# beautifulNow1992/bolt

Hardware: AMD Instinct MI355X
Metric: swap/transpose GB/s + stat-reduce GB/s, % of HBM/xGMI roofline, 1-8 GPUs (higher is better)
Workload: dtype f32; 1 GPU; C2 f32 (2000,512,512)/GPU key=time: swap((0,),(0,1)) + mean/std(axis=2); split=1, parallelism=dp1, collectives=none

## Files before the change

bolt_amd/csrc/bm_copy.hip:

```cpp
#include "bm_common.h"
#include "bm_wave.h"
#include "../../include/bolt_mi355x.h"

#include <algorithm>
#include <cstdlib>
#include <type_traits>
#include <vector>

namespace {

constexpr int kThreads = 256;
constexpr int kRcThreads = 256;
constexpr int kUnroll = 1;
constexpr uint64_t kRcGridCap = 16777208;
constexpr int64_t kDiagMinStep = 65536;
constexpr int64_t kDiagMaxRow = 4096;
constexpr int kPkTA = 128, kPkTB = 512, kPkThreads = 1024;
constexpr int kGenGridCap = 4096;
constexpr int kASpread = 32;
constexpr int64_t kRunsMaxBytes = 64;
constexpr uint64_t kMaxGrid = 0xffffffffull / 1024;

struct Diag16 {
  int on;
// ... 36 lines not shown
        const uint64_t v = g - row * vpr.d;
        int64_t so, dof;
        decomp_n<ND>(dg.on ? diag16_row(row, dg) : row, d, so, dof);
        reg[u] = __builtin_nontemporal_load(reinterpret_cast<const V *>(src + so + (int64_t)v * VB));
        doff[u] = dof + (int64_t)v * VB;
      }
    }
#pragma unroll
    for (int u = 0; u < kUnroll; ++u) {
      if (doff[u] >= 0) __builtin_nontemporal_store(reg[u], reinterpret_cast<V *>(dst + doff[u]));
    }
  }
}

struct TransDesc {
  int64_t La;
  int64_t Lb;
  int64_t sb;
  int64_t da;
  FastDiv ntB;
  FastDiv ntAB;
  uint64_t ntiles;
  Decomp batch;
  FastDiv Lb1, La1;
  int64_t sb2, da2;
  FastDiv asp;
  uint64_t aspq;
};

template <bool FUSED>
__device__ __forceinline__ int64_t brow(const TransDesc &d, int64_t b) {
  if (!FUSED) return b * d.sb;
  const int64_t hi = (int64_t)fd_div((uint64_t)b, d.Lb1);
  return (b - hi * (int64_t)d.Lb1.d) * d.sb + hi * d.sb2;
}

template <bool FUSED>
__device__ __forceinline__ int64_t arow(const TransDesc &d, int64_t a) {
  if (!FUSED) return a * d.da;
  const int64_t hi = (int64_t)fd_div((uint64_t)a, d.La1);
  return (a - hi * (int64_t)d.La1.d) * d.da + hi * d.da2;
}


struct MomOut {
  double *parts;
  int64_t nrows;
  int64_t pitch;
};
struct NoMom {};

__device__ __forceinline__ double pair_fold16(double a, double b, int lane) {
  const bool hi = lane & 8;
  double v = (hi ? b : a) + dpp_mov<0x140>(hi ? a : b);
  v += dpp_mov<0x141>(v);
  v += dpp_mov<0x4E>(v);
  v += dpp_mov<0xB1>(v);
  return v;
}

template <typename T, int TA, int TB, int VA, int VB, bool FUSED = false, typename F = void>
__global__ void __launch_bounds__(kThreads)
    k_transpose(const T *__restrict__ src, T *__restrict__ dst, TransDesc d,
                typename std::conditional<std::is_void<F>::value, NoMom, MomOut>::type mo) {
  __shared__ T tile[TB][TA + 1];
  constexpr int NVA = TA / VA;
  constexpr int RPA = kThreads / NVA;
  constexpr int NVB = TB / VB;
  constexpr int RPB = kThreads / NVB;
  static_assert(NVA <= kThreads && NVB <= kThreads, "tile row wider than the block");
  static_assert(RPA <= TB && RPB <= TA && TB % RPA == 0 && TA % RPB == 0, "tile too small for the thread layout");
  constexpr int NL = TB / RPA;
  constexpr int NS = TA / RPB;
  constexpr int RPL = (VA * (int)sizeof(T) + 3) / 4;
  constexpr int NLB = (NL * RPL <= 64) ? NL : (16 / RPL > 0 ? 16 / RPL : 1);
  static_assert(NL % NLB == 0, "load batch must divide the loads");
  const int tx = threadIdx.x % NVA, ty = threadIdx.x / NVA;
  const int ux = threadIdx.x % NVB, uy = threadIdx.x / NVB;
  const int ia = tx * VA;
  const int ib = ux * VB;
  constexpr bool MOM = !std::is_void<F>::value;
  constexpr int NSEG = NVB / 16;
  static_assert(!MOM || (!FUSED && sizeof(typename std::conditional<MOM, F, T>::type) == sizeof(T) &&
                         VA * sizeof(T) == 16 && VB * sizeof(T) == 16 && NVB % 16 == 0 && NS % 2 == 0 &&
                         3 * TA <= kThreads),
                "moments: vectorised unfused tiles of float / double only");
  __shared__ double mst[MOM ? (2 * NSEG + 1) * TA : 1];
  double p1 = 0.0, p2 = 0.0, pK = 0.0;

  for (uint64_t t = blockIdx.x; t < d.ntiles; t += gridDim.x) {
    const uint64_t bt = fd_div(t, d.ntAB);
    const uint64_t rem = t - bt * d.ntAB.d;
    uint64_t ta = fd_div(rem, d.ntB);
    uint64_t tb = rem - ta * d.ntB.d;
    if (d.asp.d > 1) {
      const uint64_t hi = fd_div(ta, d.asp);
      ta = (ta - hi * d.asp.d) * d.aspq + hi;
    }
    int64_t so, dof;
    decomp_le4(bt, d.batch, so, dof);
    const int64_t a0 = (int64_t)ta * TA, b0 = (int64_t)tb * TB;

    const T *s = src + so + a0;
    const bool fullA = (a0 + ia + VA <= d.La);
#pragma unroll
    for (int i0 = 0; i0 < NL; i0 += NLB) {
      T v[NLB][VA];
#pragma unroll
      for (int j = 0; j < NLB; ++j) {
        const int rb = ty + (i0 + j) * RPA;
        if (b0 + rb < d.Lb) {
          const T *p = s + ia + brow<FUSED>(d, b0 + rb);
          if (fullA) {
            vload_nt<T, VA>(p, v[j]);
          } else {
#pragma unroll
            for (int k = 0; k < VA; ++k) v[j][k] = (a0 + ia + k < d.La) ? p[k] : T(0);
          }
        }
      }
#pragma unroll
      for (int j = 0; j < NLB; ++j) {
        const int rb = ty + (i0 + j) * RPA;
#pragma unroll
        for (int k = 0; k < VA; ++k) tile[rb][ia + k] = v[j][k];
      }
    }
    __syncthreads();

    T *q = dst + b0;
    if constexpr (!MOM) q += dof;
    const bool fullB = (b0 + ib + VB <= d.Lb);
#pragma unroll
    for (int it = 0; it < NS; ++it) {
      const int ra = uy + it * RPB;
      if (MOM || a0 + ra < d.La) {
        T w[VB];
#pragma unroll
        for (int k = 0; k < VB; ++k) w[k] = tile[ib + k][ra];
        if (!MOM || a0 + ra < d.La) {
          T *p = q + ib;
          if constexpr (MOM) p += (dof + (a0 + ra) * d.da) * mo.pitch;
          else p += arow<FUSED>(d, a0 + ra);
          if (fullB) {
            vstore_nt<T, VB>(p, w);
          } else {
#pragma unroll
            for (int k = 0; k < VB; ++k)
              if (b0 + ib + k < d.Lb) p[k] = w[k];
          }
        }
        if constexpr (MOM) {
          const double K0 = (double)__builtin_bit_cast(F, tile[0][ra]);
          const double K = K0 - K0 == 0.0 ? K0 : 0.0;
          double s1 = 0.0, s2 = 0.0;
#pragma unroll
          for (int k = 0; k < VB; ++k) {
            const double y = b0 + ib + k < d.Lb ? (double)__builtin_bit_cast(F, w[k]) - K : 0.0;
            s1 += y;
            s2 = fma(y, y, s2);
          }
          if ((it & 1) == 0) {
            p1 = s1;
            p2 = s2;
            pK = K;
          } else {
            const int lane = threadIdx.x & 63;
            s1 = pair_fold16(p1, s1, lane);
            s2 = pair_fold16(p2, s2, lane);
            if ((lane & 7) == 0) {
              const int rr = (lane & 8) ? ra : ra - RPB, seg = ux / 16;
              mst[rr * NSEG + seg] = s1;
              mst[(TA + rr) * NSEG + seg] = s2;
              if (seg == 0) mst[2 * TA * NSEG + rr] = (lane & 8) ? K : pK;
            }
          }
        }
      }
    }
    __syncthreads();
    if constexpr (MOM) {
      const int r = threadIdx.x % TA, plane = threadIdx.x / TA;
      if (plane < 3 && a0 + r < d.La) {
        double S1 = 0.0, S2 = 0.0;
#pragma unroll
        for (int g = 0; g < NSEG; ++g) {
          S1 += mst[r * NSEG + g];
          S2 += mst[(TA + r) * NSEG + g];
        }
        const double n = (double)min((int64_t)TB, d.Lb - b0);
        const double m1 = S1 / n;
        const double m2 = fma(-S1, m1, S2);
        const int64_t row = dof + (a0 + r) * d.da;
        mo.parts[((int64_t)tb * 3 + plane) * mo.nrows + row] =
            plane == 0 ? mst[2 * TA * NSEG + r] : plane == 1 ? m1 : (m2 > 0.0 ? m2 : 0.0);
      }
    }
  }
}


template <typename T, int TA, int TB, int NT = kThreads>
__global__ void __launch_bounds__(NT)
    k_transpose_pk(const T *__restrict__ src, T *__restrict__ dst, TransDesc d) {
  constexpr int P = 4 / (int)sizeof(T);
  constexpr int VA = 16 / (int)sizeof(T);
  constexpr int TBW = TB / P;
  constexpr int NVA = TA / VA;
  constexpr int RGA = NT / NVA;
  constexpr int NL = TBW / RGA;
  constexpr int NVB = TBW / 4;
  constexpr int RPB = NT / NVB;
  constexpr int NS = TA / RPB;
  constexpr int BITS = 8 * (int)sizeof(T);
  static_assert(NL >= 1 && TBW % RGA == 0 && NS >= 1 && TA % RPB == 0, "tile too small for the thread layout");
  static_assert(NL * P * 4 <= 64, "loads in flight exceed the register budget");
  __shared__ uint32_t tile[TBW][TA + 1];
  const int tx = threadIdx.x % NVA, ty = threadIdx.x / NVA;
  const int ux = threadIdx.x % NVB, uy = threadIdx.x / NVB;
  const int ia = tx * VA;

  for (uint64_t t = blockIdx.x; t < d.ntiles; t += gridDim.x) {
    const uint64_t bt = fd_div(t, d.ntAB);
    const uint64_t rem = t - bt * d.ntAB.d;
    const uint64_t ta = fd_div(rem, d.ntB);
    uint64_t tb = rem - ta * d.ntB.d;
    int64_t so, dof;
    decomp_le4(bt, d.batch, so, dof);
    const int64_t a0 = (int64_t)ta * TA, b0 = (int64_t)tb * TB;

    const T *s = src + so + a0 + b0 * d.sb;
// ... 858 lines not shown
```

bolt_amd/csrc/bm_reduce.hip:

```cpp
#include "bm_common.h"
#include "bm_wave.h"
#include "../../include/bolt_mi355x.h"

#include <cmath>

namespace {

constexpr int kThreads = 256;
constexpr int64_t kMaxBlocks = 0xffffffffLL / kThreads;
constexpr int kColsUnroll = 8;
constexpr int64_t kColsBlocks = 2048;
constexpr int64_t kColsTcv = 64;
constexpr int64_t kColsTcvMin = 64;
constexpr int kRowsUnroll = 2;
constexpr int kIntUnroll = 8;

enum Mode {
  M_MEAN = 0, M_MOM = 1, M_FSUM = 2, M_ISUM = 3, M_OR = 4, M_MAX = 5, M_MIN = 6,
  M_FPROD = 7, M_IPROD = 8, M_LAND = 9, M_BAND = 10, M_BOR = 11, M_BXOR = 12, M_FMAX = 13, M_FMIN = 14,
  M_MEANMOM = 15
};
template <int MODE> constexpr bool mean_part() { return MODE == M_MEAN || MODE == M_MEANMOM; }
template <int MODE> constexpr bool mom_part() { return MODE == M_MOM || MODE == M_MEANMOM; }

// ... 193 lines not shown
  if (na == nb) {
    f = 0.5;
  } else {
    f = nb / n;
  }
  ma = fma(delta, f, ma);
  if (need_m2) qa = qa + qb + delta * delta * (na * f);
  na = n;
}

__device__ __forceinline__ void store_out(void *out, int64_t idx, double v, int dt) {
  switch (dt) {
    case BM_F16: ((_Float16 *)out)[idx] = (_Float16)v; break;
    case BM_F32: ((float *)out)[idx] = (float)v; break;
    default: ((double *)out)[idx] = v; break;
  }
}

__device__ __forceinline__ void store_int(void *out, int64_t idx, uint64_t v, int dt) {
  switch (dt) {
    case BM_BOOL:
    case BM_U8:
    case BM_I8: ((uint8_t *)out)[idx] = (uint8_t)v; break;
    case BM_U16:
    case BM_I16:
    case BM_F16: ((uint16_t *)out)[idx] = (uint16_t)v; break;
    case BM_U32:
    case BM_I32:
    case BM_F32: ((uint32_t *)out)[idx] = (uint32_t)v; break;
    default: ((uint64_t *)out)[idx] = v; break;
  }
}

__device__ __forceinline__ double finish(int stat, double mean, double m2, double n) {
  if (stat == BM_STAT_MEAN) return mean;
  const double var = n > 0.0 ? m2 / n : __builtin_nan("");
  return stat == BM_STAT_VAR ? var : sqrt(var);
}

constexpr int kFinalMoments = 2;
struct Sink {
  void *out;
  int out_dtype;
  int stat;
  int final_out;
  double *p0;
  double *p1;
  double *p2;
  int shifted;
  void *om, *ov, *os;
  double *k0, *k1;
};

__device__ __forceinline__ void emit_kept(const Sink &sk, int64_t idx, double mean_y, double m2, double P) {
  sk.k0[idx] = P + mean_y;
  sk.k1[idx] = m2 > 0.0 ? m2 : 0.0;
}

__device__ __forceinline__ void emit_mom(const Sink &sk, int64_t idx, int64_t e, int64_t c, double n,
                                         double mean_y, double m2, double P) {
  m2 = m2 > 0.0 ? m2 : 0.0;
  if (sk.k0) emit_kept(sk, idx, mean_y, m2, P);
  if (sk.final_out == kFinalMoments) {
    if (sk.om) store_out(sk.om, idx, n > 0.0 ? P + mean_y : 0.0, sk.out_dtype);
    if (sk.ov) store_out(sk.ov, idx, finish(BM_STAT_VAR, 0.0, m2, n), sk.out_dtype);
    if (sk.os) store_out(sk.os, idx, finish(BM_STAT_STD, 0.0, m2, n), sk.out_dtype);
    return;
  }
  if (sk.final_out) {
    store_out(sk.out, idx, finish(sk.stat, 0.0, m2, n), sk.out_dtype);
    return;
  }
  sk.p0[idx] = sk.shifted ? mean_y : P + mean_y;
  sk.p1[idx] = m2;
  if (sk.shifted && c == 0) sk.p2[e] = P;
}

template <int MODE>
__device__ __forceinline__ void emit(const Sink &sk, int64_t e, double n, double mean, double m2,
                                     uint64_t u) {
  if (bit_mode<MODE>()) {
    if (sk.final_out) store_int(sk.out, e, u, sk.out_dtype);
    else ((uint64_t *)sk.p0)[e] = u;
  } else if (facc_mode<MODE>()) {
    if (sk.final_out) store_out(sk.out, e, mean, sk.out_dtype);
    else sk.p0[e] = mean;
  } else {
    if (sk.final_out) store_out(sk.out, e, finish(sk.stat, mean, m2, n), sk.out_dtype);
    else {
      sk.p0[e] = mean;
      if (MODE == M_MOM) sk.p1[e] = m2;
    }
  }
}

__device__ __forceinline__ uint64_t xcd_block() {
  uint64_t bid = blockIdx.x;
  const uint64_t g8 = gridDim.x / 8 * 8;
  if (bid < g8) bid = (bid % 8) * (g8 / 8) + bid / 8;
  return bid;
}

struct ColsDesc {
  int64_t O, R, I;
  int64_t rchunk;
  int64_t nchunks;
  int32_t tcv;
  int32_t nph;
  FastDiv ntc;
  int64_t tile0;
};

template <typename T, int VEC, int MODE>
__global__ void __launch_bounds__(kThreads)
// ... 1005 lines not shown
  if (p.nchunks <= 1) {
    int rc = launch_main(mode, dt, p, src, O, R, P, I, sk, st);
    if (rc) return rc;
    return check_launch(who);
  }
  const size_t need = ws_bytes_for(mode, p, nout);
  if (!ws || ws_bytes < need) {
    bm_set_error("%s: workspace too small (%zu < %zu)", who, ws_bytes, need);
    return BM_E_WS;
  }
  double *w0 = (double *)ws;
  double *w1 = w0 + (size_t)p.nchunks * nout;
  Sink part = sk;
  part.final_out = 0;
  part.p0 = w0;
  part.p1 = w1;
  part.p2 = w1 + (size_t)p.nchunks * nout;
  part.shifted = mode == M_MOM;
  int rc = launch_main(mode, dt, p, src, O, R, P, I, part, st);
  if (rc) return rc;
  CombDesc cd{};
  cd.nout = nout;
  cd.nparts = p.nchunks;
  cd.part_stride = nout;
  cd.R = R;
  cd.rchunk = p.rchunk;
  cd.explicit_counts = 0;
  cd.int_sums = mode == M_MOM && !is_float(dt) && dtype_size(dt) <= 2;
  cd.pivots = mode == M_MOM && !cd.int_sums;
  rc = launch_combine(mode, dt, w0, w1, cd, sk, st);
  if (rc) return rc;
  return check_launch(who);
}

__global__ void __launch_bounds__(kThreads)
    k_red_merge_tiles(const double *__restrict__ parts, int64_t nparts, int64_t tb, int64_t R, int64_t nrows,
                      double *__restrict__ state) {
  const int64_t step = (int64_t)gridDim.x * kThreads;
  for (int64_t e = (int64_t)blockIdx.x * kThreads + threadIdx.x; e < nrows; e += step) {
    const double K0 = parts[e];
    double n = 0.0, m = 0.0, q = 0.0;
    for (int64_t p = 0; p < nparts; ++p) {
      const double nb = (double)(min(R, (p + 1) * tb) - p * tb);
      const double *pp = parts + 3 * p * nrows + e;
      chan(n, m, q, nb, (pp[0] - K0) + pp[nrows], pp[2 * nrows], true);
    }
    m += K0;
    if (m != m) {
      double s = 0.0;
      for (int64_t p = 0; p < nparts; ++p) s += parts[3 * p * nrows + e] + parts[(3 * p + 1) * nrows + e];
      m = s;
    }
    state[e] = m;
    state[nrows + e] = q > 0.0 ? q : 0.0;
  }
}

}

int bm_merge_tile_moments(const double *parts, int64_t nparts, int64_t tb, int64_t R, int64_t nrows,
                          double *state, hipStream_t stream) {
  int64_t g = cdiv(nrows, kThreads);
  if (g > 4096) g = 4096;
  k_red_merge_tiles<<<(int)g, kThreads, 0, stream>>>(parts, nparts, tb, R, nrows, state);
  return check_launch("bm_copy_strided_moments");
}

extern "C" int bm_reduce_workspace_bytes(int stat, int in_dtype, int64_t O, int64_t R, int64_t I,
                                         size_t *bytes) {
  if (!bytes) { bm_set_error("bm_reduce_workspace_bytes: null out"); return BM_E_ARG; }
  int rc = check_args(stat, in_dtype, O, R, I, "bm_reduce_workspace_bytes");
  if (rc) return rc;
  const int mode = mode_of(stat, in_dtype);
  const size_t a = ws_bytes_for(mode, plan_reduce(in_dtype, O, R, I, nullptr, R), O * I);
  const size_t b = ws_bytes_for(mode, plan_reduce(in_dtype, O, R, I, (const void *)1, R), O * I);
  *bytes = a > b ? a : b;
  return BM_OK;
}

namespace {
int reduce_to_out(int stat, const void *src, int in_dtype, int64_t O, int64_t R, int64_t I, int64_t P,
                  void *out, int out_dtype, void *workspace, size_t workspace_bytes, void *stream,
                  const char *who) {
  int rc = check_args(stat, in_dtype, O, R, I, who);
  if (rc) return rc;
  if (!src || !out) { bm_set_error("%s: null pointer", who); return BM_E_ARG; }
  const int mode = mode_of(stat, in_dtype);
  if (!out_dtype_ok(stat, mode, in_dtype, out_dtype)) {
    bm_set_error("%s: out_dtype %d does not fit stat %d on dtype %d (float for statistics and "
                 "float sums / products, bool for logical and / or, else the input dtype)",
                 who, out_dtype, stat, in_dtype);
    return BM_E_ARG;
  }
  if (is_float(in_dtype) && (mode == M_BAND || mode == M_BOR || mode == M_BXOR)) {
    bm_set_error("%s: bitwise reductions need an integer or bool dtype", who);
    return BM_E_ARG;
  }
  Sink sk{};
  sk.out = out;
  sk.out_dtype = out_dtype;
  sk.stat = stat;
  sk.final_out = 1;
  return run_reduce(stat, src, in_dtype, O, R, I, sk, workspace, workspace_bytes,
                    (hipStream_t)stream, who, P);
}
}

// ... 185 lines not shown
```

bolt_amd/csrc/bm_wave.h:

```cpp
#pragma once

#include "bm_common.h"

template <typename T> __device__ __forceinline__ double to_f64(T x) { return (double)x; }
template <> __device__ __forceinline__ double to_f64<_Float16>(_Float16 x) { return (double)(float)x; }

template <int CTRL, typename V> __device__ __forceinline__ V dpp_mov(V v) {
  static_assert(sizeof(V) == 8, "64-bit lane values");
  const uint64_t u = __builtin_bit_cast(uint64_t, v);
  const uint32_t lo = (uint32_t)__builtin_amdgcn_update_dpp(0, (int)(uint32_t)u, CTRL, 0xf, 0xf, false);
  const uint32_t hi = (uint32_t)__builtin_amdgcn_update_dpp(0, (int)(uint32_t)(u >> 32), CTRL, 0xf, 0xf, false);
  return __builtin_bit_cast(V, ((uint64_t)hi << 32) | lo);
}
template <typename V, typename F> __device__ __forceinline__ V wave_fold(V v, int lane, F op) {
  V p = dpp_mov<0xB1>(v);
  v = (lane & 1) ? op(p, v) : op(v, p);
  p = dpp_mov<0x4E>(v);
  v = (lane & 2) ? op(p, v) : op(v, p);
  p = dpp_mov<0x141>(v);
  v = (lane & 4) ? op(p, v) : op(v, p);
  p = dpp_mov<0x140>(v);
  v = (lane & 8) ? op(p, v) : op(v, p);
  p = dpp_mov<0x142>(v);
  if (lane & 16) v = op(p, v);
  p = dpp_mov<0x143>(v);
  if (lane & 32) v = op(p, v);
  return v;
}
constexpr int kFoldLane = 63;
template <int L> __device__ __forceinline__ double lane_of(double v) {
  const uint64_t u = __builtin_bit_cast(uint64_t, v);
  const uint32_t lo = (uint32_t)__builtin_amdgcn_readlane((int)(uint32_t)u, L);
  const uint32_t hi = (uint32_t)__builtin_amdgcn_readlane((int)(uint32_t)(u >> 32), L);
  return __builtin_bit_cast(double, ((uint64_t)hi << 32) | lo);
}
__device__ __forceinline__ double lane0_of(double v) { return lane_of<0>(v); }

constexpr uint64_t kRedXcdSkew = 37;
__device__ __forceinline__ uint64_t rows_block() {
  uint64_t bid = blockIdx.x;
  const uint64_t g8 = gridDim.x / 8 * 8;
  if (bid < g8) {
    const uint64_t E = g8 / 8;
    bid = (bid % 8) * E + (bid / 8 + (bid % 8) * kRedXcdSkew) % E;
  }
  return bid;
}
```

bolt_amd/mi355x/array.py:

```python
import collections
import functools
import os

import numpy as np

from bolt_amd.mi355x import _lib, reduction
from bolt_amd.mi355x._ops import backend_for, dtype_code
from bolt_amd.base import BoltArray
from bolt_amd.mi355x.context import local_shape
from bolt_amd.mi355x.dist import all_gather_bytes, concat_rows_sharded, gather_to_host, permute_sharded, redistribute_rows, select_sharded, _empty
from bolt_amd.mi355x.transfer import to_device, to_host
from bolt_amd.local import BoltArrayLocal
from bolt_amd.mi355x.plan import getplan, check_plan, padded_strides, swap_perm, swap_shape, reduce_layout
from bolt_amd.utils import tupleize, argpack, inshape, istransposeable, isreshapeable

_STAT_CODES = {'mean': _lib.STAT_MEAN, 'variance': _lib.STAT_VAR, 'stdev': _lib.STAT_STD}


def _ufunc_stats():
    import operator
    return {operator.add: _lib.STAT_SUM, np.add: _lib.STAT_SUM,
            np.maximum: _lib.STAT_MAX, np.minimum: _lib.STAT_MIN,
            operator.mul: _lib.STAT_PROD, np.multiply: _lib.STAT_PROD,
            np.logical_and: _lib.STAT_LAND, np.logical_or: _lib.STAT_LOR,
# ... 86 lines not shown
    if rows < 2:
        return None
    sstr = [1] * len(shape)
    for k in range(len(shape) - 2, -1, -1):
        sstr[k] = sstr[k + 1] * shape[k + 1]
    return P, rows, list(new_shape), [sstr[p] for p in perm], _padded_strides(new_shape, P)


_DEVICE_BYTES = {}


def _pitch_fits(pp, es, device):
    if device.type != "cuda":
        return True
    import torch
    P, rows, oshape = pp[0], pp[1], pp[2]
    need = rows * (P + oshape[-1]) * es
    idx = device.index if device.index is not None else torch.cuda.current_device()
    total = _DEVICE_BYTES.get(idx)
    if total is None:
        total = _DEVICE_BYTES[idx] = torch.cuda.get_device_properties(idx).total_memory
    if need * 8 <= total:
        return True
    free = torch.cuda.mem_get_info(idx)[0] + torch.cuda.memory_reserved(idx) - torch.cuda.memory_allocated(idx)
    return need <= free


_padded_strides = padded_strides


@functools.lru_cache(maxsize=1024)
def _aligned_vshape_of(shape, split, axis):
    tokeys = [a - split for a in axis if a >= split]
    tovalues = [a for a in range(split) if a not in axis]
    if not (tokeys or tovalues):
        return None
    ref = swap_shape(shape, split, tovalues, tokeys)
    if ref is None:
        return None
    vs = ref[0][ref[1]:]
    kept = tuple(d for i, d in enumerate(shape) if i not in set(axis))
    return None if vs == kept else vs


KEEP_MOMENTS = os.environ.get("BOLT_AMD_KEEP_MOMENTS", "1") != "0"
_KEEP_MIN_BYTES = 256 << 20
_KEEP_STATE_DIV = 64
_KEEP_COLS = False

FUSE_SWAP_MOMENTS = os.environ.get("BOLT_AMD_FUSE_SWAP_MOMENTS", "1") != "0"
_FUSE_SWAP_MIN_BYTES = 256 << 20
_FUSE_SWAP_STATE_DIV = 64

Kept = collections.namedtuple('Kept', ('state', 'count', 'nlaunch', 'drop', 'serves_mean'))

Stats = collections.namedtuple('Stats', ('count', 'mean', 'var', 'std'))
_STATS_FIELDS = reduction.STATS_FIELDS
_STATS_NAMES = {'mean': 'mean', 'var': 'var', 'variance': 'var', 'std': 'std', 'stdev': 'std'}
_STAT_AXES = {}


class BoltArrayMI355X(BoltArray):

    _metadata = {
        '_shape': None,
        '_split': None,
        '_dtype': None,
        '_ordered': True,
    }

    def __init__(self, data, shape=None, split=None, dtype=None, ordered=True, context=None,
                 npartitions=None):
        self._data = data
        self._shape = tuple(int(s) for s in shape)
        self._split = int(split)
        self._dtype = np.dtype(dtype)
        self._mode = 'mi355x'
        self._ordered = ordered
        self._ctx = context
        self._npartitions = npartitions

    @property
    def _constructor(self):
        return BoltArrayMI355X

    @classmethod
    def _ingest(cls, arry, permutation, shape, split, dtype, ctx, npartitions):
        import torch
        dev = ctx.device
        es = dtype.itemsize
        arry = np.ascontiguousarray(arry)
        identity = list(permutation) == list(range(len(shape)))
        lo, hi = ctx.local_bounds(shape[0])
        rowbytes = int(np.prod(shape[1:], dtype=np.int64)) * es
        if identity:
            data = to_device(arry[lo:hi].reshape(-1).view(np.uint8), dev)
        elif ctx.world_size == 1:
            full = to_device(arry.reshape(-1).view(np.uint8), dev)
            data = _empty(full.numel(), dev)
            if full.numel():
                backend_for(dev).permute(full, arry.shape, permutation, es, data)
        else:
            pshape = tuple(arry.shape[i] for i in permutation)
            inner0 = int(np.prod(pshape[1:], dtype=np.int64))
            s0, e0 = lo * (rowbytes // es), hi * (rowbytes // es)
            if e0 == s0 or inner0 == 0:
                data = _empty(0, dev)
# ... 159 lines not shown
                sstr = [pstr[p] for p in perm]
            else:
                src, sstr = self._data, None
            be = backend_for(src.device)
            R = new_shape[-1]
            if pp is not None:
                P, rows, oshape, psstr, dstr = pp
            else:
                P, oshape, dstr = R, list(new_shape), _padded_strides(new_shape, R)
                if sstr is None:
                    cstr = _padded_strides(self._shape, self._shape[-1])
                    psstr = [cstr[p] for p in perm]
            csstr = psstr if sstr is None else sstr
            st = self._swap_state(be, src.device, new_shape, es, oshape, csstr, dstr, P)
            if pp is None and sstr is None and st is None:
                return self._derive(permute_sharded(self._ctx, be, src, self._shape, perm, es), new_shape, split)
            n = rows * P if pp is not None else int(np.prod(new_shape, dtype=np.int64))
            dst = _empty(n * es, src.device)
            if st is None:
                be.copy_strided(src, 0, dst, 0, oshape, csstr, dstr, es)
                fused = False
            else:
                fused = be.copy_strided(src, 0, dst, 0, oshape, csstr, dstr, es, moments=(st[0], R, P, st[1], st[2]))
            out = self._derive_padded(dst, P, new_shape, split) if pp is not None \
                else self._derive(dst, new_shape, split)
            return out._with_swap_state(st, fused)
        else:
            es = self._dtype.itemsize
            pp = self._pitch_of(mv, es) if ROW_PITCH else None
            d = self.__dict__
            src = d["_pbuf"] if "_pbuf" in d else self._data
            data = permute_sharded(self._ctx, backend_for(src.device), src, self._shape, perm, es,
                                   src_pitch=d.get("_pitch"), out_pitch=None if pp is None else pp[0])
            if pp is not None:
                return self._derive_padded(data, pp[0], new_shape, split)
        return self._derive(data, new_shape, split)

    def _swap_state(self, be, dev, new_shape, es, oshape, sstr, dstr, pitch):
        if not FUSE_SWAP_MOMENTS or self._dtype.kind != 'f' or es not in (4, 8) or self._dtype.byteorder == '>' \
                or len(new_shape) < 2 \
                or not getattr(be, "fuses_swap_moments", False):
            return None
        rows = int(np.prod(new_shape[:-1], dtype=np.int64))
        nbytes = rows * new_shape[-1] * es
        if not rows or nbytes <= _FUSE_SWAP_MIN_BYTES or 16 * rows > nbytes // _FUSE_SWAP_STATE_DIV:
            return None
        code = dtype_code(self._dtype)
        if not be.copy_moments_plan(oshape, sstr, dstr, es, code, new_shape[-1], pitch, rows)[3]:
            return None
        return code, rows, _empty(be.state_bytes(_lib.STAT_VAR, code, rows), dev)

    def _with_swap_state(self, st, fused):
        if fused:
            self.__dict__["_kept"] = {(len(self._shape) - 1,): Kept(st[2], self._shape[-1], st[1], None, True)}
        return self

    def _pitch_of(self, mv, es):
        key = (mv, es)
        pp = _PITCH_PLANS.get(key, False)
        if pp is False:
            pp = _pitch_plan(mv, self._shape, es)
            if len(_PITCH_PLANS) > 4096:
                _PITCH_PLANS.clear()
            _PITCH_PLANS[key] = pp
        if pp is not None and not _pitch_fits(pp, es, self._device):
            return None
        return pp

    def chunk(self, size="150", axis=None, padding=None):
        if type(size) is not str:
            size = tupleize((size))
        axis = tupleize((axis))
        padding = tupleize((padding))
        from bolt_amd.mi355x.chunk import ChunkedArrayMI355X
        return ChunkedArrayMI355X._from_array(self, size, axis, padding)

    def swap(self, kaxes, vaxes, size="150"):
        try:
            raw = (self._shape, self._split, self._dtype, kaxes, vaxes, size)
            hit = _SWAP_PLANS.get(raw)
        except TypeError:
            raw = hit = None
        if hit is None:
            try:
                key = (self._shape, self._split, self._dtype, tuple(int(k) for k in tupleize(kaxes)),
                       tuple(int(v) for v in tupleize(vaxes)), size if type(size) is str else tupleize(size))
                hash(key)
            except (TypeError, ValueError):
                key = None
            hit = _SWAP_PLANS.get(key) if key is not None else None
            if hit is None:
                plan = self._swap_plan(kaxes, vaxes, size)
                if plan is None:
                    hit = _NOOP
                else:
                    mv = _move_plan(self._shape, *plan[:2])
                    ref = swap_shape(self._shape, self._split, *plan[2:])
                    hit = (mv, ref[0] if ref is not None and ref[0] != mv[2] else None)
            if len(_SWAP_PLANS) > 4096:
                _SWAP_PLANS.clear()
            for k in (key, raw):
                if k is not None:
                    _SWAP_PLANS[k] = hit
        if hit is _NOOP:
            return self
        mv, squeezed = hit
        out = self._move(mv)
# ... 392 lines not shown
        src = reduction.source(self, plan, stat in _MOMENTS)
        buf, O, R, I, pitch, nlaunch, drop, every = src
        dev = buf.device
        be = backend_for(dev)
        if every:
            mean, var = reduction.every_axis_moments(be, src, stat, code)
            v = mean if stat == _lib.STAT_MEAN else var if stat == _lib.STAT_VAR else np.sqrt(var)
            return np.asarray(v, dtype=np.float64).astype(out_dtype).reshape(plan.out_shape), out_dtype
        single = plan.world == 1
        if single or 0 not in axes:
            run = nlaunch and plan.nloc
            outs = reduction.outputs(be, dev, out_dtype, 1, nlaunch, single and run)
            if run:
                st = self._keep_state(be, dev, axes, stat, code, nlaunch, O * R * I, I > 1)
                fn, last = (be.reduce_rows, pitch) if pitch != R else (be.reduce, I)
                if st is None:
                    fn(stat, buf, code, O, R, last, outs[0][0], ocode)
                elif fn(stat, buf, code, O, R, last, outs[0][0], ocode, state=st):
                    self.__dict__.setdefault("_kept", {})[axes] = Kept(st, R, nlaunch, drop, False)
            return reduction.finish(outs, dev, plan, out_dtype, 1, nlaunch, drop, None if single else self._ctx)[0], \
                out_dtype
        if plan.nout == 0:
            return np.empty(plan.out_shape, out_dtype), out_dtype
        states, counts = reduction.sharded_states(self._ctx, be, dev, plan, stat, src)
        outs = reduction.outputs(be, dev, out_dtype, 1, plan.nout, False)
        be.reduce_combine(stat, code, states, counts, plan.nout, outs[0][0], ocode)
        return reduction.finish(outs, dev, plan, out_dtype, 1, plan.nout)[0], out_dtype

    def _kept_for(self, axes, stat):
        held = self.__dict__.get("_kept")
        entry = held.get(axes) if held else None
        if entry is not None and stat in _MOMENTS \
                and (entry.serves_mean or (KEEP_MOMENTS and stat != _lib.STAT_MEAN)):
            return entry
        return None

    def _keep_state(self, be, dev, axes, stat, code, nlaunch, nread, cols):
        if not KEEP_MOMENTS or stat not in _MOMENTS or self._dtype.kind != 'f' or self._ctx.world_size != 1 \
                or not getattr(be, "keeps_moments", False):
            return None
        if cols and not _KEEP_COLS:
            return None
        held = self.__dict__.get("_kept")
        if held and axes in held:
            return None
        nbytes = nread * self._dtype.itemsize
        if nbytes <= _KEEP_MIN_BYTES or 16 * nlaunch > nbytes // _KEEP_STATE_DIV:
            return None
        return _empty(be.state_bytes(_lib.STAT_VAR, code, nlaunch), dev)

    def _from_kept(self, entry, stat, plan, out_dtype, ocode):
        dev = entry.state.device
        be = backend_for(dev)
        outs = reduction.outputs(be, dev, out_dtype, 1, entry.nlaunch, True)
        with np.errstate(all="ignore"):
            be.reduce_combine(stat, plan.code, entry.state, [entry.count], entry.nlaunch, outs[0][0], ocode)
            return reduction.finish(outs, dev, plan, out_dtype, 1, entry.nlaunch, entry.drop)[0]

    def _reduced_moments(self, axis, want):
        plan, out_dtype, ocode = reduction.plan_for(self, axis, _lib.STAT_VAR)
        src = reduction.source(self, plan)
        nlaunch, drop, every = src[5:]
        dev = src.buf.device
        be = backend_for(dev)
        code, k = plan.code, len(want)
        single = plan.world == 1
        if every:
            mean, var = reduction.every_axis_moments(be, src, _lib.STAT_VAR, code)
            vals = {'mean': mean, 'var': var, 'std': np.sqrt(var)}
            return dict((f, np.asarray(vals[f], dtype=np.float64).astype(out_dtype).reshape(plan.out_shape))
                        for f in want)
        if single or 0 not in plan.axes:
            run = nlaunch and plan.nloc
            outs = reduction.outputs(be, dev, out_dtype, k, nlaunch, single and run)
            if run:
                reduction.launch_moments(be, src, self._dtype.itemsize, code, ocode, want, outs[0])
            res = reduction.finish(outs, dev, plan, out_dtype, k, nlaunch, drop, None if single else self._ctx)
        elif plan.nout == 0:
            return dict((f, np.empty(plan.out_shape, out_dtype)) for f in want)
        else:
            states, counts = reduction.sharded_states(self._ctx, be, dev, plan, _lib.STAT_VAR, src)
            outs = reduction.outputs(be, dev, out_dtype, k, plan.nout, False)
            reduction.combine_moments(be, code, ocode, want, states, counts, plan.nout, outs[0])
            res = reduction.finish(outs, dev, plan, out_dtype, k, plan.nout)
        return dict(zip(want, res))

    def stats(self, axis=None, keepdims=False, names=_STATS_FIELDS):
        if isinstance(names, str):
            names = (names,)
        try:
            asked = set(_STATS_NAMES[n] for n in names)
        except (KeyError, TypeError):
            raise ValueError("stats: names must be among %s, got %r" % (sorted(_STATS_NAMES), names))
        if not asked:
            raise ValueError("stats: no statistic asked for")
        want = tuple(f for f in _STATS_FIELDS if f in asked)
        ax = tupleize(list(range(len(self.shape))) if axis is None else axis)
        inshape(self.shape, ax)
        count = self._nrecords(ax)
        if len(want) == 1:
            one = getattr(self, want[0])(axis=axis, keepdims=keepdims)
            return Stats(count=count, **dict((f, one if f == want[0] else None) for f in _STATS_FIELDS))
        if count == 0:
            res = dict((f, 0.0 if f == 'mean' else float('nan')) for f in want)
        else:
            vs = self._aligned_vshape(ax)
            res = self._reduced_moments(ax, want)
            for f in want:
                arr = res[f]
                if vs is not None:
# ... 312 lines not shown
```

bolt_amd/mi355x/reduction.py:

```python
import collections

import numpy as np

from bolt_amd.mi355x import _lib
from bolt_amd.mi355x._ops import backend_for, dtype_code
from bolt_amd.mi355x.dist import all_gather_bytes, _empty
from bolt_amd.mi355x.plan import padded_strides, reduce_layout, stat_dtype
from bolt_amd.mi355x.transfer import SMALL as HOST_RESULT_MAX, finish_host_result, host_result, to_host

MOMENTS = (_lib.STAT_MEAN, _lib.STAT_VAR, _lib.STAT_STD)
_KEEP_DTYPE = (_lib.STAT_SUM, _lib.STAT_MAX, _lib.STAT_MIN, _lib.STAT_PROD, _lib.STAT_BAND,
               _lib.STAT_BOR, _lib.STAT_BXOR, _lib.STAT_FMAX, _lib.STAT_FMIN)
STANDARDIZE = 'standardize'
STATS_FIELDS = ('mean', 'var', 'std')

Plan = collections.namedtuple('Plan', ('axes', 'lshape', 'shape', 'dtype', 'world', 'out_shape',
                                       'perm', 'O', 'R', 'I', 'nloc', 'nout', 'code', 'outs'))
_PLANS = {}

Source = collections.namedtuple('Source', ('buf', 'O', 'R', 'I', 'pitch', 'nlaunch', 'drop', 'every'))
_tuple_new = tuple.__new__


def plan_for(arr, axis, stat):
    lshape = arr._local_shape
    key = (lshape, tuple(axis), arr._dtype, arr._shape, arr._ctx.world_size)
    plan = _PLANS.get(key)
    if plan is None:
        axes = tuple(sorted(set(int(a) for a in axis)))
        kept = [i for i in range(len(lshape)) if i not in axes]
        perm, O, R, I = reduce_layout(lshape, axes)
        plan = Plan(axes, lshape, arr._shape, arr._dtype, key[4], tuple(arr._shape[i] for i in kept),
                    perm, O, R, I, int(np.prod(lshape, dtype=np.int64)),
                    int(np.prod([lshape[i] for i in kept], dtype=np.int64)), dtype_code(arr._dtype), {})
        if len(_PLANS) > 4096:
            _PLANS.clear()
        _PLANS[key] = plan
    out = plan.outs.get(stat)
    if out is None:
        if stat in _KEEP_DTYPE:
            dt = plan.dtype
        elif stat in (_lib.STAT_LAND, _lib.STAT_LOR):
            dt = np.dtype(bool)
        else:
            dt = stat_dtype(plan.dtype, (1,) if stat == STANDARDIZE else plan.out_shape)
        out = plan.outs[stat] = (dt, dtype_code(dt))
    return plan, out[0], out[1]


def source(arr, plan, moments=True, compact=False):
    d = arr.__dict__
    pbuf = d.get("_pbuf")
    lshape, perm, O, R, I, nloc = plan.lshape, plan.perm, plan.O, plan.R, plan.I, plan.nloc
    if pbuf is None and perm is None:
        return _tuple_new(Source, (d["_data"], O, R, I, R, plan.nout, None, False))
    if pbuf is not None and perm is None:
        P, Rl, single = d["_pitch"], lshape[-1], plan.world == 1
        if I == 1 and R == Rl and (nloc if single else 0 not in plan.axes):
            return Source(pbuf, O, R, 1, P, plan.nout, None, False)
        if single and nloc and not compact:
            if I > 1 and I % Rl == 0:
# ... 6 lines not shown
    if perm is not None:
        dev = arr._device
        buf = _empty(nloc * es, dev)
        if pbuf is not None:
            pstr = padded_strides(lshape, d["_pitch"])
            pshape = [lshape[p] for p in perm]
            backend_for(dev).copy_strided(pbuf, 0, buf, 0, pshape, [pstr[p] for p in perm],
                                          padded_strides(pshape, pshape[-1]), es)
        elif nloc:
            backend_for(dev).permute(arr._data, lshape, perm, es, buf)
    elif pbuf is not None and compact:
        buf = _empty(nloc * es, pbuf.device)
        if nloc:
            backend_for(pbuf.device).copy_strided(pbuf, 0, buf, 0, [nloc // lshape[-1], lshape[-1]],
                                                  [d["_pitch"], 1], [lshape[-1], 1], es)
    else:
        buf = arr._data
    return Source(buf, O, R, I, R, plan.nout, None, False)


def sharded_states(ctx, be, dev, plan, stat, src):
    if plan.world > _lib.MAX_COMBINE_PARTS:
        raise NotImplementedError("reductions over the sharded axis merge at most %d ranks (got %d)"
                                  % (_lib.MAX_COMBINE_PARTS, plan.world))
    sbytes = be.state_bytes(stat, plan.code, plan.nout)
    state = _empty(sbytes, dev)
    if plan.nloc:
        be.reduce_state(stat, src.buf, plan.code, src.O, src.R, src.I, state)
    else:
        state.zero_()
    per = int(np.prod([plan.shape[i] for i in plan.axes if i != 0], dtype=np.int64))
    counts = [(hi - lo) * per for lo, hi in ctx.bounds(plan.shape[0])]
    return all_gather_bytes(ctx, state, [sbytes] * plan.world), counts


def gathered_sizes(ctx, plan, itemsize, k=1):
    return [k * int(np.prod((hi - lo,) + plan.out_shape[1:], dtype=np.int64)) * itemsize
            for lo, hi in ctx.bounds(plan.shape[0])]


def outputs(be, dev, out_dtype, k, n, host_ok):
    nb = n * out_dtype.itemsize
    host = host_result(be, k * nb, dev) if host_ok else None
    if host is None and host_ok and nb <= HOST_RESULT_MAX < k * nb:
        hosts = [host_result(be, nb, dev) for _ in range(k)]
        if all(h is not None for h in hosts):
            return hosts, hosts, None
    if host is not None:
        return ([host] if k == 1 else [host[j * nb:(j + 1) * nb] for j in range(k)]), host, None
    buf = _empty(k * nb, dev)
    return ([buf] if k == 1 else [buf[j * nb:(j + 1) * nb] for j in range(k)]), None, buf


def finish(outs, dev, plan, out_dtype, k, n, drop=None, ctx=None):
    _, host, buf = outs
    pshape = plan.out_shape if drop is None else drop[:3]
    shape = pshape if k == 1 else (k, n)
    if ctx is not None:
        isz = out_dtype.itemsize
        sizes = gathered_sizes(ctx, plan, isz, k)
        flat = to_host(all_gather_bytes(ctx, buf, sizes), out_dtype, (-1,))
        parts, off = [], 0
        for s in sizes:
            m = s // isz
            parts.append(flat[off:off + m].reshape(k, m // k))
            off += m
        host = np.concatenate(parts, axis=1)
        if k == 1:
            host = host.reshape(pshape)
    elif host is None:
        host = to_host(buf, out_dtype, shape)
    elif type(host) is list:
        host = [finish_host_result(host[0], dev, out_dtype, (n,))] + [h.numpy().view(out_dtype) for h in host[1:]]
    else:
        host = finish_host_result(host, dev, out_dtype, shape)
    rows = [host] if k == 1 else [host[j].reshape(pshape) for j in range(k)]
    if drop is None:
        return rows
    return [np.ascontiguousarray(full[:, :, :drop[3]]).reshape(plan.out_shape) for full in rows]


def _slots(planes, want):
    slots = [None, None, None]
    for t, f in zip(planes, want):
        slots[STATS_FIELDS.index(f)] = t
    return tuple(slots)


def combine_moments(be, code, ocode, want, states, counts, nout, planes):
    if hasattr(be, "reduce_combine_moments"):
        return be.reduce_combine_moments(code, states, counts, nout, _slots(planes, want), ocode)
    om, ov, osd = _slots(planes, want)
    with np.errstate(all="ignore"):
        if om is not None:
            means = states.view(len(counts), 2, nout * 8)[:, 0, :].contiguous().view(-1)
            be.reduce_combine(_lib.STAT_MEAN, code, means, counts, nout, om, ocode)
        if ov is not None:
            be.reduce_combine(_lib.STAT_VAR, code, states, counts, nout, ov, ocode)
        if osd is not None:
            be.reduce_combine(_lib.STAT_STD, code, states, counts, nout, osd, ocode)


def launch_moments(be, src, es, code, ocode, want, planes):
    buf, O, R, I, pitch = src[:5]
    if hasattr(be, "reduce_moments"):
        return be.reduce_moments(buf, code, O, R, I, pitch, _slots(planes, want), ocode)
    if pitch != R:
        dense = _empty(O * R * es, buf.device)
        be.copy_strided(buf, 0, dense, 0, [O, R], [pitch, 1], [R, 1], es)
        buf = dense
    state = _empty(be.state_bytes(_lib.STAT_VAR, code, O * I), buf.device)
    with np.errstate(all="ignore"):
        be.reduce_state(_lib.STAT_VAR, buf, code, O, R, I, state)
    combine_moments(be, code, ocode, want, state, [R], O * I, planes)


def merge_equal_counts(planes, Rl, nrows):
    means = planes[0, :Rl]
    mean = means.mean()
    if len(planes) < 2:
        return mean, None
    return mean, (planes[1, :Rl].sum() + nrows * np.square(means - mean).sum()) / (nrows * Rl)


def every_axis_moments(be, src, stat, code):
    nrows, P, Rl = src.R, src.I, src.drop[3]
    state = _empty(be.state_bytes(stat, code, P), src.buf.device)
    be.reduce_state(stat, src.buf, code, 1, nrows, P, state)
# ... 2 lines not shown
```

bolt_amd/mi355x/transfer.py:

```python
from concurrent.futures import ThreadPoolExecutor

import numpy as np

CHUNK = 64 << 20
SMALL = 8 << 20
THREADS = 8
H2D_DIRECT = True

ZERO_COPY = True

_POOL = None


def _pool():
    global _POOL
    if _POOL is None:
        _POOL = ThreadPoolExecutor(max_workers=THREADS, thread_name_prefix="bolt-amd-copy")
    return _POOL


def _par_copy(dst, src):
    n = src.size
    if n < (4 << 20):
        dst[:] = src
# ... 77 lines not shown
        return
    bufs = staging if staging is not None else staging_buffers()
    evs = [torch.cuda.Event(), torch.cuda.Event()]
    starts = list(range(0, n, chunk))
    for i, lo in enumerate(starts):
        hi = min(n, lo + chunk)
        k = i % 2
        bufs[k][:hi - lo].copy_(src(lo, hi, k), non_blocking=True)
        evs[k].record(stream)
        if i > 0:
            plo = starts[i - 1]
            phi = min(n, plo + chunk)
            evs[1 - k].synchronize()
            _par_copy(out[plo:phi], bufs[1 - k].numpy()[:phi - plo])
    lo = starts[-1]
    evs[(len(starts) - 1) % 2].synchronize()
    _par_copy(out[lo:n], bufs[(len(starts) - 1) % 2].numpy()[:n - lo])


def host_result(backend, nbytes, device):
    if not ZERO_COPY or device.type != "cuda" or not 0 < nbytes <= SMALL:
        return None
    writable = getattr(backend, "host_writable", None)
    if writable is None:
        return None
    import torch
    host = torch.empty(nbytes, dtype=torch.uint8, pin_memory=True)
    key = (host.data_ptr(), nbytes, device.index)
    ok = _WRITABLE.get(key)
    if ok is None:
        ok = bool(writable(host))
        if len(_WRITABLE) > 1024:
            _WRITABLE.clear()
        _WRITABLE[key] = ok
    return host if ok else None


_WRITABLE = {}


_STREAMS = {}


def current_stream(device):
    import torch
    idx = device.index if device.index is not None else torch.cuda.current_device()
    raw = torch._C._cuda_getCurrentRawStream(idx)
    s = _STREAMS.get(idx)
    if s is None or s.cuda_stream != raw:
        s = _STREAMS[idx] = torch.cuda.current_stream(device)
    return s


def finish_host_result(host, device, dtype, shape):
    current_stream(device).synchronize()
    return host.numpy().view(np.dtype(dtype)).reshape(shape)
```

Measured before the change: 10120 GB/s.

## Split moment transpose path, use full-lane DPP, and precompute paired stat ahead

The fused swap+moments kernel path is restructured. Rows are processed in explicit even/odd pairs through a lambda, with an unmasked specialisation chosen when the tile is fully in bounds. DPP folds switch to mov_dpp with bound_ctrl so every lane has a source. On the host side, asking for mean or std from kept state also queues the other statistic's combine kernel with an event, so the second request can wait on an event rather than synchronise the whole stream. NaN propagation in m2 output is also changed, which alters semantics for non-finite inputs.

```diff
diff --git a/bolt_amd/csrc/bm_copy.hip b/bolt_amd/csrc/bm_copy.hip
--- a/bolt_amd/csrc/bm_copy.hip
+++ b/bolt_amd/csrc/bm_copy.hip
@@ -112,10 +112,10 @@
 
 __device__ __forceinline__ double pair_fold16(double a, double b, int lane) {
   const bool hi = lane & 8;
-  double v = (hi ? b : a) + dpp_mov<0x140>(hi ? a : b);
-  v += dpp_mov<0x141>(v);
-  v += dpp_mov<0x4E>(v);
-  v += dpp_mov<0xB1>(v);
+  double v = (hi ? b : a) + dpp_mov_all<0x140>(hi ? a : b);
+  v += dpp_mov_all<0x141>(v);
+  v += dpp_mov_all<0x4E>(v);
+  v += dpp_mov_all<0xB1>(v);
   return v;
 }
 
@@ -146,7 +146,6 @@
                          3 * TA <= kThreads),
                 "moments: vectorised unfused tiles of float / double only");
   __shared__ double mst[MOM ? (2 * NSEG + 1) * TA : 1];
-  double p1 = 0.0, p2 = 0.0, pK = 0.0;
 
   for (uint64_t t = blockIdx.x; t < d.ntiles; t += gridDim.x) {
     const uint64_t bt = fd_div(t, d.ntAB);
@@ -191,17 +190,15 @@
     T *q = dst + b0;
     if constexpr (!MOM) q += dof;
     const bool fullB = (b0 + ib + VB <= d.Lb);
-#pragma unroll
-    for (int it = 0; it < NS; ++it) {
-      const int ra = uy + it * RPB;
-      if (MOM || a0 + ra < d.La) {
-        T w[VB];
-#pragma unroll
-        for (int k = 0; k < VB; ++k) w[k] = tile[ib + k][ra];
-        if (!MOM || a0 + ra < d.La) {
-          T *p = q + ib;
-          if constexpr (MOM) p += (dof + (a0 + ra) * d.da) * mo.pitch;
-          else p += arow<FUSED>(d, a0 + ra);
+    if constexpr (!MOM) {
+#pragma unroll
+      for (int it = 0; it < NS; ++it) {
+        const int ra = uy + it * RPB;
+        if (a0 + ra < d.La) {
+          T w[VB];
+#pragma unroll
+          for (int k = 0; k < VB; ++k) w[k] = tile[ib + k][ra];
+          T *p = q + ib + arow<FUSED>(d, a0 + ra);
           if (fullB) {
             vstore_nt<T, VB>(p, w);
           } else {
@@ -210,33 +207,60 @@
               if (b0 + ib + k < d.Lb) p[k] = w[k];
           }
         }
-        if constexpr (MOM) {
-          const double K0 = (double)__builtin_bit_cast(F, tile[0][ra]);
-          const double K = K0 - K0 == 0.0 ? K0 : 0.0;
-          double s1 = 0.0, s2 = 0.0;
-#pragma unroll
-          for (int k = 0; k < VB; ++k) {
-            const double y = b0 + ib + k < d.Lb ? (double)__builtin_bit_cast(F, w[k]) - K : 0.0;
-            s1 += y;
-            s2 = fma(y, y, s2);
-          }
-          if ((it & 1) == 0) {
-            p1 = s1;
-            p2 = s2;
-            pK = K;
+      }
+    } else {
+      const int na = (int)min((int64_t)TA, d.La - a0), nb = (int)min((int64_t)TB, d.Lb - b0);
+      constexpr bool UNMASKED = sizeof(tile) > (48 << 10);
+      const auto row_sums = [&](auto full, int it, T *p, double &s1, double &s2, double &K) {
+        constexpr bool FULL = decltype(full)::value;
+        const int ra = uy + it * RPB;
+        T w[VB];
+#pragma unroll
+        for (int k = 0; k < VB; ++k) w[k] = tile[ib + k][ra];
+        if (FULL || uy < na - it * RPB) {
+          if (FULL || ib <= nb - VB) {
+            vstore_nt<T, VB>(p, w);
           } else {
-            const int lane = threadIdx.x & 63;
-            s1 = pair_fold16(p1, s1, lane);
-            s2 = pair_fold16(p2, s2, lane);
-            if ((lane & 7) == 0) {
-              const int rr = (lane & 8) ? ra : ra - RPB, seg = ux / 16;
-              mst[rr * NSEG + seg] = s1;
-              mst[(TA + rr) * NSEG + seg] = s2;
-              if (seg == 0) mst[2 * TA * NSEG + rr] = (lane & 8) ? K : pK;
-            }
+#pragma unroll
+            for (int k = 0; k < VB; ++k)
+              if (ib < nb - k) p[k] = w[k];
           }
         }
-      }
+        const F k0 = __builtin_bit_cast(F, tile[0][ra]);
+        K = (double)(__builtin_isfinite(k0) ? k0 : F(0));
+        s1 = 0.0;
+        s2 = 0.0;
+#pragma unroll
+        for (int k = 0; k < VB; ++k) {
+          const double y = (FULL || ib < nb - k) ? (double)__builtin_bit_cast(F, w[k]) - K : 0.0;
+          s1 += y;
+          s2 = fma(y, y, s2);
+        }
+      };
+      const auto row_pairs = [&](auto full) {
+        const int lane = threadIdx.x & 63;
+        T *const p0 = q + ib + (dof + (a0 + uy) * d.da) * mo.pitch;
+        const int64_t pstep = (int64_t)RPB * d.da * mo.pitch;
+#pragma unroll
+        for (int it = 0; it < NS; it += 2) {
+          const int ra = uy + it * RPB;
+          double e1, e2, eK, o1, o2, oK;
+          row_sums(full, it, p0 + it * pstep, e1, e2, eK);
+          row_sums(full, it + 1, p0 + (it + 1) * pstep, o1, o2, oK);
+          const double K = (lane & 8) ? oK : eK;
+          const double s1 = pair_fold16(e1, o1, lane);
+          const double s2 = pair_fold16(e2, o2, lane);
+          if ((lane & 7) == 0) {
+            const int rr = (lane & 8) ? ra + RPB : ra, seg = ux / 16;
+            mst[rr * NSEG + seg] = s1;
+            mst[(TA + rr) * NSEG + seg] = s2;
+            if (seg == 0) mst[2 * TA * NSEG + rr] = K;
+          }
+        }
+      };
+      const int64_t slack = (d.Lb - b0 - TB) | (d.La - a0 - TA);
+      if (UNMASKED && (int32_t)((uint64_t)slack >> 32) >= 0) row_pairs(std::true_type{});
+      else row_pairs(std::false_type{});
     }
     __syncthreads();
     if constexpr (MOM) {
diff --git a/bolt_amd/csrc/bm_reduce.hip b/bolt_amd/csrc/bm_reduce.hip
--- a/bolt_amd/csrc/bm_reduce.hip
+++ b/bolt_amd/csrc/bm_reduce.hip
@@ -269,14 +269,18 @@
   double *k0, *k1;
 };
 
+__device__ __forceinline__ double m2_out(double m2, double mean) {
+  return mean - mean == 0.0 ? (m2 > 0.0 ? m2 : 0.0) : __builtin_nan("");
+}
+
 __device__ __forceinline__ void emit_kept(const Sink &sk, int64_t idx, double mean_y, double m2, double P) {
   sk.k0[idx] = P + mean_y;
-  sk.k1[idx] = m2 > 0.0 ? m2 : 0.0;
+  sk.k1[idx] = m2_out(m2, P + mean_y);
 }
 
 __device__ __forceinline__ void emit_mom(const Sink &sk, int64_t idx, int64_t e, int64_t c, double n,
                                          double mean_y, double m2, double P) {
-  m2 = m2 > 0.0 ? m2 : 0.0;
+  m2 = m2_out(m2, P + mean_y);
   if (sk.k0) emit_kept(sk, idx, mean_y, m2, P);
   if (sk.final_out == kFinalMoments) {
     if (sk.om) store_out(sk.om, idx, n > 0.0 ? P + mean_y : 0.0, sk.out_dtype);
@@ -1388,7 +1392,7 @@
       m = s;
     }
     state[e] = m;
-    state[nrows + e] = q > 0.0 ? q : 0.0;
+    state[nrows + e] = m2_out(q, m);
   }
 }
 
diff --git a/bolt_amd/csrc/bm_wave.h b/bolt_amd/csrc/bm_wave.h
--- a/bolt_amd/csrc/bm_wave.h
+++ b/bolt_amd/csrc/bm_wave.h
@@ -10,6 +10,14 @@
   const uint64_t u = __builtin_bit_cast(uint64_t, v);
   const uint32_t lo = (uint32_t)__builtin_amdgcn_update_dpp(0, (int)(uint32_t)u, CTRL, 0xf, 0xf, false);
   const uint32_t hi = (uint32_t)__builtin_amdgcn_update_dpp(0, (int)(uint32_t)(u >> 32), CTRL, 0xf, 0xf, false);
+  return __builtin_bit_cast(V, ((uint64_t)hi << 32) | lo);
+}
+template <int CTRL, typename V> __device__ __forceinline__ V dpp_mov_all(V v) {
+  static_assert(sizeof(V) == 8, "64-bit lane values");
+  static_assert(CTRL == 0xB1 || CTRL == 0x4E || CTRL == 0x141 || CTRL == 0x140, "a source lane for every lane");
+  const uint64_t u = __builtin_bit_cast(uint64_t, v);
+  const uint32_t lo = (uint32_t)__builtin_amdgcn_mov_dpp((int)(uint32_t)u, CTRL, 0xf, 0xf, true);
+  const uint32_t hi = (uint32_t)__builtin_amdgcn_mov_dpp((int)(uint32_t)(u >> 32), CTRL, 0xf, 0xf, true);
   return __builtin_bit_cast(V, ((uint64_t)hi << 32) | lo);
 }
 template <typename V, typename F> __device__ __forceinline__ V wave_fold(V v, int lane, F op) {
diff --git a/bolt_amd/mi355x/array.py b/bolt_amd/mi355x/array.py
--- a/bolt_amd/mi355x/array.py
+++ b/bolt_amd/mi355x/array.py
@@ -162,7 +162,11 @@
 _FUSE_SWAP_MIN_BYTES = 256 << 20
 _FUSE_SWAP_STATE_DIV = 64
 
-Kept = collections.namedtuple('Kept', ('state', 'count', 'nlaunch', 'drop', 'serves_mean'))
+FINISH_AHEAD = os.environ.get("BOLT_AMD_FINISH_AHEAD", "1") != "0"
+_AHEAD_OF = {_lib.STAT_MEAN: _lib.STAT_STD, _lib.STAT_STD: _lib.STAT_MEAN}
+
+Kept = collections.namedtuple('Kept', ('state', 'count', 'nlaunch', 'drop', 'serves_mean', 'ahead'))
+Kept.__new__.__defaults__ = (None,)
 
 Stats = collections.namedtuple('Stats', ('count', 'mean', 'var', 'std'))
 _STATS_FIELDS = reduction.STATS_FIELDS
@@ -428,7 +432,7 @@
 
     def _with_swap_state(self, st, fused):
         if fused:
-            self.__dict__["_kept"] = {(len(self._shape) - 1,): Kept(st[2], self._shape[-1], st[1], None, True)}
+            self.__dict__["_kept"] = {(len(self._shape) - 1,): Kept(st[2], self._shape[-1], st[1], None, True, {})}
         return self
 
     def _pitch_of(self, mv, es):
@@ -927,10 +931,25 @@
     def _from_kept(self, entry, stat, plan, out_dtype, ocode):
         dev = entry.state.device
         be = backend_for(dev)
-        outs = reduction.outputs(be, dev, out_dtype, 1, entry.nlaunch, True)
+        ahead = entry.ahead
+        queued = ahead.pop(stat, None) if ahead else None
         with np.errstate(all="ignore"):
+            if queued is not None:
+                return reduction.finish(queued.take(), dev, plan, out_dtype, 1, entry.nlaunch, entry.drop,
+                                        event=queued.event)[0]
+            outs = reduction.outputs(be, dev, out_dtype, 1, entry.nlaunch, True)
             be.reduce_combine(stat, plan.code, entry.state, [entry.count], entry.nlaunch, outs[0][0], ocode)
-            return reduction.finish(outs, dev, plan, out_dtype, 1, entry.nlaunch, entry.drop)[0]
+            event = None
+            other = _AHEAD_OF.get(stat)
+            if FINISH_AHEAD and other is not None and ahead is not None and not ahead and outs[1] is not None:
+                odt, oc = reduction.plan_for(self, plan.axes, other)[1:]
+                outs2 = reduction.outputs(be, dev, odt, 1, entry.nlaunch, True)
+                if outs2[1] is not None:
+                    event = reduction.record_event(dev)
+                    be.reduce_combine(other, plan.code, entry.state, [entry.count], entry.nlaunch, outs2[0][0], oc)
+                    ahead[other] = reduction.Queued(outs2, reduction.record_event(dev))
+                    ahead[None] = True
+            return reduction.finish(outs, dev, plan, out_dtype, 1, entry.nlaunch, entry.drop, event=event)[0]
 
     def _reduced_moments(self, axis, want):
         plan, out_dtype, ocode = reduction.plan_for(self, axis, _lib.STAT_VAR)
diff --git a/bolt_amd/mi355x/reduction.py b/bolt_amd/mi355x/reduction.py
--- a/bolt_amd/mi355x/reduction.py
+++ b/bolt_amd/mi355x/reduction.py
@@ -6,7 +6,7 @@
 from bolt_amd.mi355x._ops import backend_for, dtype_code
 from bolt_amd.mi355x.dist import all_gather_bytes, _empty
 from bolt_amd.mi355x.plan import padded_strides, reduce_layout, stat_dtype
-from bolt_amd.mi355x.transfer import SMALL as HOST_RESULT_MAX, finish_host_result, host_result, to_host
+from bolt_amd.mi355x.transfer import SMALL as HOST_RESULT_MAX, current_stream, finish_host_result, host_result, to_host
 
 MOMENTS = (_lib.STAT_MEAN, _lib.STAT_VAR, _lib.STAT_STD)
 _KEEP_DTYPE = (_lib.STAT_SUM, _lib.STAT_MAX, _lib.STAT_MIN, _lib.STAT_PROD, _lib.STAT_BAND,
@@ -119,7 +119,32 @@
     return ([buf] if k == 1 else [buf[j * nb:(j + 1) * nb] for j in range(k)]), None, buf
 
 
-def finish(outs, dev, plan, out_dtype, k, n, drop=None, ctx=None):
+def record_event(dev):
+    import torch
+    ev = torch.cuda.Event()
+    ev.record(current_stream(dev))
+    return ev
+
+
+class Queued(object):
+    __slots__ = ("outs", "event")
+
+    def __init__(self, outs, event):
+        self.outs, self.event = outs, event
+
+    def take(self):
+        outs, self.outs = self.outs, None
+        return outs
+
+    def __del__(self):
+        if self.outs is not None:
+            try:
+                self.event.synchronize()
+            except Exception:
+                pass
+
+
+def finish(outs, dev, plan, out_dtype, k, n, drop=None, ctx=None, event=None):
     _, host, buf = outs
     pshape = plan.out_shape if drop is None else drop[:3]
     shape = pshape if k == 1 else (k, n)
@@ -140,7 +165,7 @@
     elif type(host) is list:
         host = [finish_host_result(host[0], dev, out_dtype, (n,))] + [h.numpy().view(out_dtype) for h in host[1:]]
     else:
-        host = finish_host_result(host, dev, out_dtype, shape)
+        host = finish_host_result(host, dev, out_dtype, shape, event)
     rows = [host] if k == 1 else [host[j].reshape(pshape) for j in range(k)]
     if drop is None:
         return rows
diff --git a/bolt_amd/mi355x/transfer.py b/bolt_amd/mi355x/transfer.py
--- a/bolt_amd/mi355x/transfer.py
+++ b/bolt_amd/mi355x/transfer.py
@@ -153,6 +153,9 @@
     return s
 
 
-def finish_host_result(host, device, dtype, shape):
-    current_stream(device).synchronize()
+def finish_host_result(host, device, dtype, shape, event=None):
+    if event is not None:
+        event.synchronize()
+    else:
+        current_stream(device).synchronize()
     return host.numpy().view(np.dtype(dtype)).reshape(shape)
```

Measured after the change: 10430 GB/s, median of 6. 3.1% higher.
